# JuliaCrypto/ToyFHE.jl

Measured on AMD Instinct MI355X. Metric: ciphertext-mul/s (BFV ct*ct + relinearize, N=2^14, L=8 RNS), higher is better.
Workload: dtype u64; 1 GPU; BFV N=2^14, L=8 RNS limbs (50-bit primes), extension basis 17 limbs, t=65537, ciphertext-mul + relinearize (RNS-digit keyswitch), bit-exact; batch_per_gpu=1024, global_batch=1024

## Files before the change

toyfhe.jl_amd/csrc/bfv_api.inc:

```

struct tfhe_bfv_plan {
    tfhe_ctx *small = nullptr, *big = nullptr;
    limb_sel_t sel_s, sel_b;
    u64 t = 0;
    bfv_tab_t tab;
    bfv_tab_t* tab_dev = nullptr;
    std::vector<void*> allocs;
    int chunk = 256;
    void* ws = nullptr;
    size_t ws_bytes = 0;
    bool relin_ok = false;
    bfv_fast_tab_t* fast_dev = nullptr;
    int fast_ns = 0, fast_np = 0;
    bool fast_narrow = false;
    bool use_fast = true;
    hipEvent_t order_ev = nullptr;
};

namespace {

int upload(tfhe_bfv_plan* p, const std::vector<u64>& v, const u64** out) {
    void* d = nullptr;
    hipError_t e = devalloc::malloc_retry(&d, std::max<size_t>(8, v.size() * 8));
    if (e != hipSuccess) return fail(TFHE_E_HIP, "hipMalloc: %s", hipGetErrorString(e));
// ... 187 lines not shown
    if (p->big && p->big->stream) hipStreamSynchronize(p->big->stream);
    if (p->small && p->small->stream && (!p->big || p->small->stream != p->big->stream)) hipStreamSynchronize(p->small->stream);
    if (p->order_ev) hipEventDestroy(p->order_ev);
    for (void* d : p->allocs) hipFree(d);
    if (p->tab_dev) hipFree(p->tab_dev);
    if (p->fast_dev) hipFree(p->fast_dev);
    if (p->ws) hipFree(p->ws);
    delete p;
    return TFHE_OK;
}

int tfhe_bfv_plan_set_chunk(tfhe_bfv_plan* p, int chunk) {
    if (!p || chunk < 0) return fail(TFHE_E_BADARG, "bad argument");
    p->chunk = chunk ? chunk : 256;
    return TFHE_OK;
}

int tfhe_bfv_plan_set_variant(tfhe_bfv_plan* p, int variant) {
    if (!p || variant < 0 || variant > 1) return fail(TFHE_E_BADARG, "variant must be 0 (auto) or 1 (general kernels)");
    p->use_fast = (variant == 0);
    return TFHE_OK;
}

int tfhe_bfv_expand(tfhe_bfv_plan* p, const uint64_t* src, uint64_t* dst, int64_t count) {
    if (!p || !src || !dst || count < 0) return fail(TFHE_E_BADARG, "bad argument");
    int rc = stream_order(p, p->small, p->big);
    if (!rc) rc = launch_expand(p, src, dst, count);
    if (!rc) rc = stream_order(p, p->big, p->small);
    return rc;
}
int tfhe_bfv_contract(tfhe_bfv_plan* p, const uint64_t* src, uint64_t* dst, int64_t count) {
    if (!p || !src || !dst || count < 0) return fail(TFHE_E_BADARG, "bad argument");
    int rc = stream_order(p, p->small, p->big);
    if (!rc) rc = launch_contract(p, src, dst, count);
    if (!rc) rc = stream_order(p, p->big, p->small);
    return rc;
}

static int bfv_mul_impl(tfhe_bfv_plan* p, const u64* evk, int n_digits, const u64* c1, const u64* c2, u64* out, int64_t batch) {
    if (!p || !c1 || !c2 || !out || batch < 0) return fail(TFHE_E_BADARG, "bad argument");
    const size_t N = (size_t)p->big->N;
    const int ns = p->tab.ns, nb = p->tab.nb;
    const bool relin = evk != nullptr;
    if (relin) {
        if (!p->relin_ok) return fail(TFHE_E_UNSUPPORTED, "relinearisation needs ℛ = limbs 0..ns-1 of the small context");
        if (n_digits < ns) return fail(TFHE_E_PARAMS_MISMATCH, "evaluation key has %d components, need %d", n_digits, ns);
    }
    const int64_t chunk = std::max<int64_t>(1, std::min<int64_t>(batch, p->chunk));
    const bool prelift = relin && p->fast_dev && p->use_fast && p->fast_narrow && ks_prelift_ok(p->small, ns);
    const size_t ntt_tmp = p->big->logN > 14 ? (size_t)chunk * 4 * nb * N * 8 : 0;
    (void)ntt_tmp;
    void* ws = nullptr;
    const size_t scr_rows = (size_t)2 * std::max(256, p->big->num_cus);
    int rc = plan_ws(p, ((size_t)chunk * (7 * (size_t)nb + (relin ? 3 * (size_t)ns : 0)) + scr_rows) * N * 8, &ws);
    if (rc) return rc;
    u64* E = (u64*)ws;
    u64* T = E + (size_t)chunk * 4 * nb * N;
    u64* R = T + (size_t)chunk * 3 * nb * N;
    u64* SCR = R + (relin ? (size_t)chunk * 3 * ns * N : 0);
    for (int64_t b0 = 0; b0 < batch; b0 += chunk) {
        const int64_t nct = std::min(chunk, batch - b0);
        const u64* a = c1 + (size_t)b0 * 2 * ns * N;
        const u64* b = c2 + (size_t)b0 * 2 * ns * N;
        rc = stream_order(p, p->small, p->big);
        if (rc) return rc;
        if (!relin) {
            rc = bfv_mul_chunk(p, a, b, out + (size_t)b0 * 3 * ns * N, nct, E, T, SCR);
            if (rc) return rc;
        } else {
            rc = bfv_mul_chunk(p, a, b, R, nct, E, T, SCR, prelift);
            if (!rc) rc = stream_order(p, p->big, p->small);
            if (rc) return rc;
            rc = keyswitch_impl(p->small, ns, ns, 0, evk, R, 3, out + (size_t)b0 * 2 * ns * N, nct, 0, false, prelift);
            if (rc) return rc;
        }
    }
    return relin ? TFHE_OK : stream_order(p, p->big, p->small);
}

int tfhe_bfv_mul(tfhe_bfv_plan* p, const uint64_t* c1, const uint64_t* c2, uint64_t* out, int64_t batch) {
    return bfv_mul_impl(p, nullptr, 0, c1, c2, out, batch);
}
int tfhe_bfv_mul_relin(tfhe_bfv_plan* p, const uint64_t* evk, int n_digits, const uint64_t* c1, const uint64_t* c2, uint64_t* out, int64_t batch) {
    if (!evk) return fail(TFHE_E_BADARG, "null evaluation key");
    return bfv_mul_impl(p, evk, n_digits, c1, c2, out, batch);
}

}
```

toyfhe.jl_amd/csrc/kernels.h:

```cpp
#pragma once
#include <hip/hip_runtime.h>
#include <type_traits>
#include "bfv_core.h"
#include "bfv_fast.h"
#include "lazy_sum.h"
#include "ntt_core.h"

typedef u64 u64x2_t __attribute__((ext_vector_type(2)));

#ifndef TFHE_NTT_WAVES
#define TFHE_NTT_WAVES 2
#endif

__device__ __forceinline__ u32 fresh_tid() {
    u32 t = threadIdx.x;
    asm volatile("" : "+v"(t));
    return t;
}

struct limb_sel_t {
    int n;
    int idx[TFHE_MAX_LIMBS];
};

// ... 67 lines not shown
        return item < nitems ? item : ~0u;
    }
    const u32 per = (nitems + 7u) >> 3, nslots = grid >> 3, xcd = wg & 7u, slot = wg >> 3;
    const u32 k = it * nslots + slot, idx = xcd * per + k;
    if (k >= per || idx >= nitems) return ~0u;
    const u32 B = nitems / nb, j = idx / B, b = idx - j * B;
    return b * nb + j;
}
__device__ __forceinline__ u32 dense_mask(u32 limbs, u32 mask) { return (limbs & 1u) ? 0u : mask; }
__device__ __forceinline__ u32 dense_count(u32 nitems, int x, u32 limbs, u32 mask) {
    return mask ? ((((nitems >> x) / limbs) * (u32)__popc(mask)) << x) : nitems;
}
__device__ __forceinline__ u32 dense_item(u32 d, int x, u32 limbs, u32 mask) {
    if (!mask || d == ~0u) return d;
    const u32 nact = (u32)__popc(mask), sb = d & ((1u << x) - 1u), pld = d >> x, g = pld / nact, a = pld % nact;
    u32 m = mask;
    for (u32 i = 0; i < a; i++) m &= m - 1u;
    return ((g * limbs + (u32)__ffs((int)m) - 1u) << x) | sb;
}
template <class A, int LOGB, int LOGT, int IOMODE>
__global__ __launch_bounds__(1 << LOGT, TFHE_NTT_WAVES) void k_ntt_fwd_block(const u64* __restrict__ src, u64* __restrict__ dst,
                                                              const ntt_limb_t* __restrict__ LT, limb_sel_t sel, int x,
                                                              u32 nitems, ntt_io_t io) {
    extern __shared__ __attribute__((aligned(16))) u64 lds[];
    const size_t ntot = (size_t)1 << (LOGB + x);
    const u32 dmask = dense_mask((u32)sel.n, io.limb_mask), dn = dense_count(nitems, x, (u32)sel.n, dmask), niter = (dn + gridDim.x - 1) / gridDim.x;
    bool first = true;
    for (u32 it = 0; it < niter; it++) {
        const u32 item = dense_item(xcd_walk_item(it, blockIdx.x, gridDim.x, x, dn), x, (u32)sel.n, dmask);
        if (item == ~0u) continue;
        const u32 sb = item & ((1u << x) - 1), pl = item >> x;
        u32 srow = pl, drow = pl, j = pl % (u32)sel.n;
        lift_t lf;
        const lift_t* lift = nullptr;
        if constexpr (IOMODE == 1) {
            const u32 per_ct = io.level * io.nw, b = pl / per_ct, rem = pl % per_ct, i = rem / io.nw;
            j = rem % io.nw;
            srow = (b * io.polys + io.polys - 1) * io.level + i;
            const ntt_limb_t& Li = LT[sel.idx[i]];
            const ntt_limb_t& Lj = LT[sel.idx[j]];
            lf.qi = Li.q; lf.half = Li.q >> 1; lf.qj = Lj.q; lf.bj = Lj.br;
            if (io.lift_unsigned) lf.qi = lf.half = ~0ull;
            lift_wide_consts<A>(lf);
            lift = &lf;
        }
        if (io.limb_mask && !((io.limb_mask >> j) & 1u)) continue;
        const typename A::ctx C = A::make(LT[sel.idx[j]]);
        if (!first) __syncthreads();
        first = false;
        fwd_schedule<A, LOGB, LOGT, 0>(lds, src + srow * ntot + ((size_t)sb << LOGB), dst + drow * ntot, C, fresh_tid(),
                                       (1u << x) + sb, x, brev_bits(sb, x), lift);
    }
}
template <class T>
__device__ __forceinline__ void pin_vgpr(T& x) { asm volatile("" : "+v"(x)); }
__device__ __forceinline__ void order_after(u32& idx, u64 v) { asm volatile("" : "+v"(idx) : "v"(v)); }
#define TFHE_WAIT_VM0() asm volatile("s_waitcnt vmcnt(0)" ::: "memory")
template <int LOGB, int LOGT>
struct row_prefetcher {
    static constexpr int E = 1 << (LOGB - LOGT);
    u64* raw;
    const u64* g;
    bool on;
    __device__ __forceinline__ void operator()(int before, int after, int total) const {
        const int lo2 = 2 * E * before / total, hi2 = 2 * E * after / total;
        const int lo = lo2 < E ? lo2 : E, hi = hi2 < E ? hi2 : E;
        if (hi > lo && on) {
#pragma unroll
            for (int i = lo; i < hi; i++) raw[i] = g[(size_t)i << LOGT];
        }
    }
};
template <class A, int LOGB, int LOGT>
__global__ __launch_bounds__(1 << LOGT, TFHE_NTT_WAVES) void k_ntt_fwd_pf(const u64* __restrict__ src, u64* __restrict__ dst,
                                                           const ntt_limb_t* __restrict__ LT, limb_sel_t sel, u32 nitems) {
    extern __shared__ __attribute__((aligned(16))) u64 lds[];
    constexpr int K1 = pass_k_fwd(LOGB, LOGT, 0), K2 = pass_k_fwd(LOGB, LOGT, K1), K3 = LOGB - K1 - K2;
    static_assert(K3 >= 1 && pass_k_fwd(LOGB, LOGT, K1 + K2) == K3, "three-pass schedule expected");
    typedef pgeom<LOGB, LOGT, K1, K2> G2;
    typedef pgeom<LOGB, LOGT, K1 + K2, K3> G3;
    static_assert(G2::SETS == 1, "middle pass: one register set");
    constexpr int E = G3::E;
    u32 item = blockIdx.x;
    if (item >= nitems) return;
    u64 raw[E];
    fwd_load_data<LOGB, LOGT, 0, K1, true, false>(raw, lds, src + ((size_t)item << LOGB), threadIdx.x);
    for (bool first = true;; first = false) {
        const u32 tid = fresh_tid();
        const typename A::ctx C = A::make(LT[sel.idx[item % (u32)sel.n]]);
        u64* gdst = dst + ((size_t)item << LOGB);
        const u32 next = item + gridDim.x;
        if (!first) __syncthreads();
        typename A::tw tw2[G2::SETS * G2::NTW];
        {
            typename A::elem v[E];
            fwd_compute<A, LOGB, LOGT, 0, K1, true, false, 0>(v, raw, nullptr, C, tid, 1u);
            fwd_load_tw<A, LOGB, LOGT, K1, K2, false>(tw2, C, tid, 1u);
            fwd_store<A, LOGB, LOGT, 0, K1, false>(v, lds, nullptr, C, tid, 0, 0u);
        }
        __syncthreads();
        {
            u64 r2[E];
            typename A::elem v[E];
            fwd_load_data<LOGB, LOGT, K1, K2, false, false>(r2, lds, nullptr, tid);
#pragma unroll
            for (int i = 0; i < G2::SETS * G2::NTW; i++) pin_vgpr(tw2[i].w);
            const row_prefetcher<LOGB, LOGT> pf{raw, src + ((size_t)(next < nitems ? next : item) << LOGB) + tid, next < nitems};
            fwd_compute<A, LOGB, LOGT, K1, K2, false, false, K2, -1, row_prefetcher<LOGB, LOGT>>(v, r2, tw2, C, tid, 1u, nullptr, pf);
// ... 1163 lines not shown
            u64x2_t p1 = {0, 0}, p2 = {0, 0};
            if (i0) {
                p1 = *s1p; p2 = *s2p;
                if (pairs) { const u64x2_t a = p1, c = p2; p1.x = a.x; p1.y = c.x; p2.x = a.y; p2.y = c.y; }
            }
            acc52 s1[2] = {{p1[0], 0, 0}, {p1[1], 0, 0}}, s2[2] = {{p2[0], 0, 0}, {p2[1], 0, 0}};
            u64x2_t dv[DCH];
#pragma unroll
            for (int ii = 0; ii < DCH; ii++)
                if (i0 + ii < A.level) dv[ii] = *(const u64x2_t*)(dig + (((size_t)b * A.level + i0 + ii) * A.nw + j) * n + k);
#pragma unroll
            for (int ii = 0; ii < DCH; ii++) {
                if (i0 + ii < A.level) {
#pragma unroll
                    for (int v = 0; v < 2; v++) {
                        const u32 d0 = (u32)dv[ii][v] & 0x3ffffffu, d1 = (u32)(dv[ii][v] >> 26);
                        acc52_mac(s1[v], d0, d1, md0[ii][v], md1[ii][v]);
                        acc52_mac(s2[v], d0, d1, mk0[ii][v], mk1[ii][v]);
                    }
                }
            }
            u64x2_t r1, r2;
#pragma unroll
            for (int v = 0; v < 2; v++) {
                u64 lo, hi;
                acc52_fold(s1[v], lo, hi);
                r1[v] = barrett_reduce128(lo, hi, br);
                acc52_fold(s2[v], lo, hi);
                r2[v] = barrett_reduce128(lo, hi, br);
            }
            if constexpr (EPI) {
                if (i0 + DCH >= A.level && j < (u32)A.level) {
                    const u64x2_t x = *(const u64x2_t*)(K.epi_x + (((size_t)b * 2) * A.level + j) * n + k);
#pragma unroll
                    for (int v = 0; v < 2; v++) {
                        r1[v] = addmod(shoup_full(r1[v], A.pinv[j], br.q), x[v], br.q);
                        r2[v] = shoup_full(r2[v], A.pinv[j], br.q);
                    }
                }
            }
            if (pairs) {
                u64x2_t a, c;
                a.x = r1[0]; a.y = r2[0]; c.x = r1[1]; c.y = r2[1];
                *s1p = a;
                *s2p = c;
            } else {
                *s1p = r1;
                *s2p = r2;
            }
        }
    }
}

template <class A, int LOGB, int LOGT, bool PRELIFT = false>
__device__ __forceinline__ void fused_fwd_to_regs(u64* lds, const u64* grow, const typename A::ctx& C, bool& first,
                                                  typename A::elem* v, const lift_t* lift = nullptr) {
    constexpr int K1 = pass_k_fwd(LOGB, LOGT, 0), K2 = pass_k_fwd(LOGB, LOGT, K1), K3 = LOGB - K1 - K2;
    constexpr int E = 1 << (LOGB - LOGT);
    const u32 tid = fresh_tid();
    {
        u64 raw[E];
        fwd_load_data<LOGB, LOGT, 0, K1, true, false>(raw, lds, grow, tid);
        if (!first) __syncthreads();
        first = false;
        if constexpr (PRELIFT) {
#pragma unroll
            for (int i = 0; i < E; i++) pin_vgpr(raw[i]);
            TFHE_SCHED_FENCE();
            fwd_compute<A, LOGB, LOGT, 0, K1, false, false, 0>(v, raw, nullptr, C, tid, 1u);
        } else {
            fwd_compute<A, LOGB, LOGT, 0, K1, true, false, 0>(v, raw, nullptr, C, tid, 1u, lift);
        }
        fwd_store<A, LOGB, LOGT, 0, K1, false>(v, lds, nullptr, C, tid, 0, 0u);
    }
    __syncthreads();
    ntt_fwd_pass<A, LOGB, LOGT, K1, K2, false, false>(lds, nullptr, nullptr, C, tid, 1u, 0, 0u);
    __syncthreads();
    {
        u64 r3[E];
        fwd_load_data<LOGB, LOGT, K1 + K2, K3, false, true>(r3, lds, nullptr, tid);
        fwd_compute<A, LOGB, LOGT, K1 + K2, K3, false, true, 0>(v, r3, nullptr, C, tid, 1u);
    }
}
template <class A, int LOGB, int LOGT, bool SCALE = true, class AO = A>
__device__ __forceinline__ void fused_inv_from_regs(u64* lds, typename A::elem* v, u64* gdst, const typename A::ctx& C, const u64* addend,
                                                    u64* keep = nullptr, u32 pre = 1u) {
    constexpr int KI1 = pass_k_inv(LOGB, LOGT, LOGB);
    constexpr int E = 1 << (LOGB - LOGT);
    const u32 tid = fresh_tid();
    __syncthreads();
    constexpr int S1 = LOGB - KI1, K2 = pass_k_inv(LOGB, LOGT, S1);
    typedef pgeom<LOGB, LOGT, S1 - K2, K2> G2;
    typename A::tw tw_next[G2::SETS * G2::NTW];
    {
#pragma unroll
        for (int e = 0; e < E; e++) v[e] = fp_reduce(v[e], C.p, C.pinv);
        inv_compute<A, LOGB, LOGT, S1, KI1, true, SCALE, 0, -1, no_hook, true>(v, nullptr, nullptr, C, tid, pre);
        if constexpr (S1 - K2 != 0) inv_load_tw<A, LOGB, LOGT, S1 - K2, K2, false>(tw_next, C, tid, pre);
        inv_store<A, LOGB, LOGT, S1, KI1, true, SCALE>(v, lds, nullptr, C, tid);
    }
    __syncthreads();
    inv_schedule_ptw<A, LOGB, LOGT, S1, SCALE, AO>(lds, nullptr, gdst, C, tid, pre, addend, tw_next, keep);
}

template <class A, int LOGB, int LOGT>
__global__ __launch_bounds__(1 << LOGT) void k_ntt_inv_quad2(const u64* __restrict__ src, u64* __restrict__ dst,
                                                              const ntt_limb_t* __restrict__ LT, limb_sel_t sel, u32 nitems, u32 limb_mask) {
    extern __shared__ __attribute__((aligned(16))) u64 lds[];
    constexpr int x = 2;
    constexpr int K1 = pass_k_inv(LOGB, LOGT, LOGB), S1 = LOGB - K1;
    typedef pgeom<LOGB, LOGT, S1, K1> G1;
    constexpr int E = G1::E;
    constexpr int K2 = pass_k_inv(LOGB, LOGT, S1), KL = S1 - K2;
    static_assert(KL >= 1 && pass_k_inv(LOGB, LOGT, KL) == KL, "three-pass schedule expected");
    typedef pgeom<LOGB, LOGT, 0, KL> GL;
    static_assert(GL::SETS == 1 && GL::LO == LOGT, "last pass: element r of a thread is word tid + (r << LOGT)");
    static_assert(G1::SETS << (LOGT + K1) == 1 << LOGB, "first pass: register position e <-> point tid + (e << LOGT)");
    const size_t ntot = (size_t)1 << (LOGB + x);
// ... 62 lines not shown
                    for (int r = 0; r < E; r++) held[r] = A::out_inv_scaled(v[r], C);
                } else {
#pragma unroll
                    for (int r = 0; r < E; r++) {
                        u64x2_t ww;
                        ww.x = held[r];
                        ww.y = A::out_inv_scaled(v[r], C);
                        *(u64x2_t*)(d + ((u64)(tid + ((u32)r << LOGT)) << x)) = ww;
                    }
                }
            }
        }
    }
}

__global__ __launch_bounds__(256) void k_evk_to_f64(const u64* __restrict__ evk, u64* __restrict__ evd,
                                                     const ntt_limb_t* __restrict__ LT, ks_arg_t KA, int Lk, u32 n, int fold_ninv, int x,
                                                     u64 ginv, int pair) {
    const u32 row = blockIdx.x, j = row % (u32)KA.nw, ic = row / (u32)KA.nw;
    const ntt_limb_t& L = LT[KA.w.idx[j]];
    const u64* s = evk + ((size_t)ic * Lk + KA.w.idx[j]) * n;
    u64* d = pair ? evd + (((size_t)(ic >> 1) * KA.nw + j) * n) * 2 + (ic & 1u) : evd + (size_t)row * n;
    for (u32 k = blockIdx.y * blockDim.x + threadIdx.x; k < n; k += gridDim.y * blockDim.x) {
        double v = fp_from_u64(s[ginv ? galois_ntt_pos(k, ginv, n) : k]);
        if (fold_ninv) {
            v = fp_mulmod_c(v, L.ninv_d, L.pd, L.pinvd);
            v = v < 0.0 ? v + L.pd : v;
        }
        u64 b;
        __builtin_memcpy(&b, &v, 8);
        const size_t pos = x ? ((size_t)(k & ((1u << x) - 1u)) * (n >> x)) + (k >> x) : (size_t)k;
        d[pair ? pos * 2 : pos] = b;
    }
}
template <int LOGB, int LOGT>
constexpr size_t fused_lds_bytes() {
    return (size_t)lds_words<LOGB, LOGT>() * 8;
}
template <class A, int LOGB, int LOGT, bool PRELIFT = false, int SPMODE = 0>
__global__ __launch_bounds__(1 << LOGT) void k_ks_fused(const u64* __restrict__ evd, const u64* __restrict__ ct,
                                                         u64* __restrict__ out, const ntt_limb_t* __restrict__ LT,
                                                         ks_arg_t KA, int Lk, u32 nitems, const u64* __restrict__ tsp = nullptr,
                                                         const u64* __restrict__ zero_row = nullptr) {
    extern __shared__ __attribute__((aligned(16))) u64 lds[];
    constexpr int K1 = pass_k_fwd(LOGB, LOGT, 0), K2 = pass_k_fwd(LOGB, LOGT, K1), K3 = LOGB - K1 - K2;
    static_assert(K3 >= 1 && pass_k_fwd(LOGB, LOGT, K1 + K2) == K3, "three-pass forward schedule expected");
    constexpr int KI1 = pass_k_inv(LOGB, LOGT, LOGB);
    static_assert(KI1 == K3, "forward last pass and inverse first pass must share the register map");
    typedef pgeom<LOGB, LOGT, 0, K1> G1;
    typedef pgeom<LOGB, LOGT, K1 + K2, K3> G3;
    constexpr int E = G3::E;
    const u32 level = (u32)KA.level, polys = (u32)KA.polys, nw = (u32)KA.nw;
    const u32 add_s = polys == 3 ? 2u : 1u;
    bool first = true;
    const u32 niter = (nitems + gridDim.x - 1) / gridDim.x;
    for (u32 it = 0; it < niter; it++) {
        const u32 nper = SPMODE == 1 ? 1u : (SPMODE >= 2 ? level : nw);
        const u32 item = it * gridDim.x + blockIdx.x;
        if (item >= nitems) break;
        const u32 b = item / nper, j = SPMODE == 1 ? level : item % nper;
        const ntt_limb_t& Lj = LT[KA.w.idx[j]];
        typename A::ctx C = A::make(Lj);
        lift_t lf;
        lf.qj = Lj.q;
        lf.bj = Lj.br;
        typename A::elem acc[2][E];
#pragma unroll
        for (int e = 0; e < E; e++) acc[0][e] = acc[1][e] = 0;
        for (u32 i = 0; i < level; i++) {
            const u32 tid = fresh_tid();
            lf.qi = LT[KA.w.idx[i]].q;
            lf.half = lf.qi >> 1;
            const u64* grow = ct + ((size_t)((b * polys + polys - 1) * level + i) << LOGB);
            typename A::elem v[E];
            fused_fwd_to_regs<A, LOGB, LOGT, PRELIFT>(lds, grow, C, first, v, &lf);
            const u64x2_t* e_pair = (const u64x2_t*)(evd + ((((size_t)i * nw + j) << LOGB) << 1));
#pragma unroll
            for (int u = 0; u < G3::SETS; u++) {
                u32 c0, hi, base;
                G3::template coords<true>(tid, u, c0, hi, base);
#pragma unroll
                for (int r = 0; r < G3::R; r++) {
                    const u32 nat = (brev_bits((u32)r, K3) << (LOGB - K3)) + c0;
                    const int e = u * G3::R + r;
                    const u64x2_t kw = e_pair[nat];
                    const typename A::tw k1{A::from_lds(kw.y)}, k0{A::from_lds(kw.x)};
                    const double y = A::pre_product(v[e], C);
                    acc[0][e] += fp_mulmod_c(y, k1, C.p, C.pinv);
                    acc[1][e] += fp_mulmod_c(y, k0, C.p, C.pinv);
                }
            }
            if ((i & 7u) == 7u && i + 1 < level) {
#pragma unroll
                for (int e = 0; e < E; e++) {
                    acc[0][e] = fp_reduce(acc[0][e], C.p, C.pinv);
                    acc[1][e] = fp_reduce(acc[1][e], C.p, C.pinv);
                }
            }
        }
#pragma unroll
        for (int sidx = 0; sidx < 2; sidx++) {
            if constexpr (SPMODE >= 2) {
                C.md_pinv = (double)KA.pinv[j].w;
                C.md_c = (u32)sidx < add_s ? ct + ((size_t)((b * polys + sidx) * level + j) << LOGB) : zero_row;
                C.md_g = KA.rot_g;
                u64* gdst = out + ((size_t)((b * 2 + sidx) * level + j) << LOGB);
                typedef typename std::conditional<SPMODE == 3, ArithFpMDR, ArithFpMD>::type AOUT;
                fused_inv_from_regs<A, LOGB, LOGT, false, AOUT>(lds, acc[sidx], gdst, C, tsp + ((size_t)(b * 2 + sidx) << LOGB));
            } else if constexpr (SPMODE == 1) {
                u64* gdst = out + ((size_t)(b * 2 + sidx) << LOGB);
                fused_inv_from_regs<A, LOGB, LOGT, false>(lds, acc[sidx], gdst, C, nullptr);
            } else {
                const u64* addend = (!KA.special && (u32)sidx < add_s) ? ct + ((size_t)((b * polys + sidx) * level + j) << LOGB) : nullptr;
                u64* gdst = out + ((size_t)((b * 2 + sidx) * nw + j) << LOGB);
                fused_inv_from_regs<A, LOGB, LOGT, false>(lds, acc[sidx], gdst, C, addend);
            }
        }
    }
}

template <class A, int LOGB, int LOGT, int X>
__global__ __launch_bounds__(1 << LOGT) void k_ks_fused_sub(const u64* __restrict__ evd, const u64* __restrict__ ct,
                                                             u64* __restrict__ T, const ntt_limb_t* __restrict__ LT,
                                                             ks_arg_t KA, int Lk, u32 nitems) {
    extern __shared__ __attribute__((aligned(16))) u64 lds[];
    constexpr int K1 = pass_k_fwd(LOGB, LOGT, 0), K2 = pass_k_fwd(LOGB, LOGT, K1), K3 = LOGB - K1 - K2;
    static_assert(K3 >= 1 && pass_k_fwd(LOGB, LOGT, K1 + K2) == K3, "three-pass forward schedule expected");
    constexpr int KI1 = pass_k_inv(LOGB, LOGT, LOGB), S1 = LOGB - KI1;
// ... 671 lines not shown
```

toyfhe.jl_amd/csrc/ks_api.inc:

```

static bool ks_fused14(const tfhe_ctx* c, int Lk, int level, int special) {
    const limb_sel_t w = working_limbs(Lk, level, special);
    if (c->variant != 0) return false;
    if (c->logN == 14) return sel_fp(c, w, 0);
    if (c->logN == 13) {
        static const bool on = env_flag("TFHE_FUSED13", true);
        return on && sel_fp(c, w, 0);
    }
    if (c->logN == 16) {
        static const bool on16 = env_flag("TFHE_FUSED16", true);
        return on16 && level >= 2 && sel_fp(c, w, 2);
    }
    return c->logN == 15 && level >= 2 && sel_fp(c, w, 1);
}
static bool ks_prelift_ok(const tfhe_ctx* c, int level) {
    if (c->logN != 14 || !ks_fused14(c, level, level, 0)) return false;
    u64 lo = ~0ull, hi = 0;
    for (int j = 0; j < level; j++) { lo = std::min(lo, c->q[j]); hi = std::max(hi, c->q[j]); }
    return hi <= 2 * lo;
}
static int launch_top_lift(tfhe_ctx* c, const u64* src, u64* t, int64_t rows, const limb_sel_t& sel, const ntt_io_t& io) {
    const int x = c->logN - 14;
    const dim3 tg((unsigned)((((c->N >> x) + 255) / 256) * rows));
    return dispatch_int<1, 2>(x, [&](auto xc) {
// ... 233 lines not shown
                         : (P.fps ? k_ks_fused_sub<ArithFpS, 14, LOGT, 1> : k_ks_fused_sub<ArithFp, 14, LOGT, 1>);
        const unsigned items = (unsigned)((batch * nw) << x);
        rc = launch_prof(c, (int64_t)batch * nw * (level + 2), fk, dim3(cu_grid(c, items)), dim3(1 << LOGT), lds, key, ct, dig, c->limbs_dev, A, Lk, items);
        if (rc) return rc;
        return launch_top_tail(c, A, P.ra, dig, ct, out, batch, P.g_tail);
    }
    lanes_t outer(c, P.two_lanes);
    rc = ks_digits_fwd(c, A, ct, dig, batch);
    if (rc) return rc;
    rc = ks_inner_launch(c, A, Lk, key, dig, S, batch);
    if (rc) return rc;
    if (P.tail16) {
        const policy_split_t ps = policy_split(c, A.w);
        const u32 fpm = ps.fpmask, amask = ps.all;
        {
            lanes_t lanes(c, fpm != amask);
            lanes.use(1);
            rc = launch_subpair<ArithFp>(c, true, S, dig, batch * 2 * nw, A.w, 2, fpm == amask ? 0u : fpm);
            if (rc) return rc;
            if (fpm != amask) {
                lanes.use(0);
                ntt_io_t iw = io_plain();
                iw.limb_mask = amask & ~fpm;
                rc = launch_block_inv<ArithInt, 14>(c, S, dig, batch * 2 * nw, A.w, 2, iw);
                if (rc) return rc;
            }
        }
        outer.join();
        return launch_top_tail(c, A, P.ra, dig, ct, out, batch, P.g_tail);
    }
    outer.join();
    return ks_plain_tail(c, A, P.ra, S, ct, out, batch);
}

static int ks_check(tfhe_ctx* c, int Lk, int level, int special, const void* evk, int n_digits, const void* ct, int polys, const void* out, int64_t batch) {
    if (!c || !evk || !ct || !out) return fail(TFHE_E_BADARG, "null argument");
    if (polys != 2 && polys != 3) return fail(TFHE_E_BADARG, "keyswitch needs a 2- or 3-element ciphertext (rlwe_she.jl:318), got %d", polys);
    if (Lk < 1 || Lk > c->L) return fail(TFHE_E_LEVEL_MISMATCH, "key_limbs=%d outside [1,%d]", Lk, c->L);
    const int maxlevel = special ? Lk - 1 : Lk;
    if (level < 1 || level > maxlevel) return fail(TFHE_E_LEVEL_MISMATCH, "level=%d outside [1,%d]", level, maxlevel);
    if (n_digits < level) return fail(TFHE_E_PARAMS_MISMATCH, "evaluation key has %d components, level %d needs %d", n_digits, level, level);
    if (batch < 0) return fail(TFHE_E_BADARG, "negative batch");
    return TFHE_OK;
}
static int galois_check(const tfhe_ctx* c, u64 g) {
    if ((g & 1) == 0 || g >= 2 * (u64)c->N) return fail(TFHE_E_BADARG, "galois element must be odd and below 2N");
    return TFHE_OK;
}
static u64 inv_mod_2n(u64 g, u64 twoN) {
    u64 x = g;
    for (int i = 0; i < 6; i++) x *= 2 - g * x;
    return x & (twoN - 1);
}
static int keyswitch_impl(tfhe_ctx* c, int Lk, int level, int special, const u64* evk, const u64* ct, int polys, u64* out, int64_t batch,
                          u64 galois, bool rotate, bool prelifted = false, bool key_prepared = false) {
    if (prelifted && (rotate || special || !ks_prelift_ok(c, level))) return fail(TFHE_E_UNSUPPORTED, "internal: pre-lifted rows need the fused key switch");
    ks_plan_t P = ks_plan(c, Lk, level, special, polys, batch, ct, out, galois, rotate, prelifted, key_prepared);
    if (P.rot == KS_ROT_HOISTED) {
        const uint64_t* one[1] = {evk};
        return tfhe_rotate_many(c, Lk, level, special, one, level, 1, &galois, 1, ct, out, batch);
    }
    if (special) special_inv_table(c, Lk, level, P.ra.qlinv);
    const size_t N = P.N;
    void* ws = nullptr;
    int rc = ensure_ws(c, P.bytes(), &ws);
    if (rc) return rc;
    u64 *const S = P.region(ws, 0), *const dig = P.region(ws, P.S_rows), *const rot = P.region(ws, P.S_rows + P.dig_rows),
        *const kw = P.region(ws, P.S_rows + P.dig_rows + P.rot_rows);
    const u64 ginv = P.key_perm ? inv_mod_2n(galois, 2 * (u64)c->N) : (u64)0;
    if (P.path != KS_THREE) {
        rc = launch(c, k_evk_to_f64, row_grid((unsigned)(level * 2 * P.A.nw), N), dim3(256), 0, evk, kw, c->limbs_dev, P.A, Lk, (u32)N, c->logN <= 14 ? 1 : 0,
                    c->logN == 16 ? 2 : 0, ginv, 1);
    } else if (P.key_perm) {
        rc = launch(c, k_ntt_perm, row_grid((unsigned)(level * 2 * Lk), N), dim3(256), 0, evk, kw, ginv, (u32)N);
    }
    if (rc) return rc;
    if (P.path != KS_THREE || P.key_perm) evk = kw;
    for (int64_t b0 = 0; b0 < batch; b0 += P.chunk) {
        const int64_t nb = std::min(P.chunk, batch - b0);
        const u64* cin = ct + (size_t)b0 * polys * level * N;
        if (P.rot == KS_ROT_COPY) {
            rc = do_galois(c, cin, rot, galois, nb * polys * level, first_limbs(level));
            if (rc) return rc;
            cin = rot;
        }
        rc = ks_chunk(c, P, evk, cin, out + (size_t)b0 * 2 * level * N, nb, S, dig);
        if (rc) return rc;
    }
    return TFHE_OK;
}

int tfhe_keyswitch(tfhe_ctx* c, int Lk, int level, int special, const uint64_t* evk, int n_digits, const uint64_t* ct, int polys, uint64_t* out, int64_t batch) {
    int rc = ks_check(c, Lk, level, special, evk, n_digits, ct, polys, out, batch);
    if (rc) return rc;
    return keyswitch_impl(c, Lk, level, special, evk, ct, polys, out, batch, 0, false);
}
int tfhe_galois_key_prepare(tfhe_ctx* c, int Lk, int n_digits, uint64_t g, const uint64_t* evk, uint64_t* evk_out) {
    if (!c || !evk || !evk_out || evk == evk_out) return fail(TFHE_E_BADARG, "null or aliased argument");
    if (Lk < 1 || Lk > c->L || n_digits < 1) return fail(TFHE_E_LEVEL_MISMATCH, "key shape outside the ring");
    if (int rc = galois_check(c, g)) return rc;
    const u64 ginv = inv_mod_2n(g, 2 * (u64)c->N);
    return launch(c, k_ntt_perm, row_grid((unsigned)(n_digits * 2 * Lk), (size_t)c->N), dim3(256), 0, evk, evk_out, ginv, (u32)c->N);
}

struct rotate_many_ws_t {
    size_t per_ct, ntt_tmp;
    int64_t chunk;
    size_t bytes() const { return ntt_tmp + (size_t)chunk * per_ct; }
};
static rotate_many_ws_t rotate_many_ws(const tfhe_ctx* c, int level, int nw, int64_t batch) {
    rotate_many_ws_t W{};
    W.per_ct = ((size_t)4 * nw + (size_t)level * nw + (size_t)2 * level) * (size_t)c->N * 8;
    W.chunk = chunk_of(c, batch, 512, (size_t)8192 << 20, W.per_ct);
    W.ntt_tmp = c->logN > 14 ? (size_t)W.chunk * std::max(2, level) * nw * (size_t)c->N * 8 : 0;
    return W;
}
int tfhe_rotate_many(tfhe_ctx* c, int Lk, int level, int special, const uint64_t* const* evks, int n_digits, int prepared,
                     const uint64_t* galois, int n_rot, const uint64_t* ct, uint64_t* out, int64_t batch) {
    if (!evks || !galois || n_rot < 0) return fail(TFHE_E_BADARG, "null argument");
    if (n_rot == 0) return TFHE_OK;
    for (int r = 0; r < n_rot; r++) {
        int rc = ks_check(c, Lk, level, special, evks[r], n_digits, ct, 2, out, batch);
        if (!rc) rc = galois_check(c, galois[r]);
        if (rc) return rc;
    }
    const int nw = special ? level + 1 : level, polys = 2;
    const size_t N = (size_t)c->N;
    if (!prepared && c->logN <= 14 && ks_fused14(c, Lk, level, special)) {
        for (int r = 0; r < n_rot; r++) {
            int rc = keyswitch_impl(c, Lk, level, special, evks[r], ct, 2, out + (size_t)r * batch * 2 * level * N, batch, galois[r], true);
// ... 154 lines not shown
```

toyfhe.jl_amd/csrc/ntt_core.h:

```cpp
#pragma once
#include "fp64arith.h"
#include "modarith.h"

#if defined(__HIP_DEVICE_COMPILE__)
#define TFHE_SCHED_FENCE() asm volatile("" ::: "memory")
#else
#define TFHE_SCHED_FENCE() ((void)0)
#endif

struct alignas(16) twd_t {
    u64 w, wp;
};
TFHE_HD tw_t as_tw(const twd_t& t) { return tw_t{t.w, t.wp}; }
TFHE_HD tw_t ld_tw(const twd_t* tab, u32 i) {
#if defined(__HIP_DEVICE_COMPILE__)
    typedef __attribute__((address_space(1))) const twd_t* gptr_t;
    const gptr_t g = (gptr_t)tab;
    return tw_t{g[i].w, g[i].wp};
#else
    return tw_t{tab[i].w, tab[i].wp};
#endif
}

template <int LOGB, int LOGT>
TFHE_HD u32 lds_phi(u32 j) {
    if (LOGB - LOGT == 5) return j + 2u * (j >> 6) + (j >> 10);
    return j + 4u * (j >> 6) + (j >> 9);
}
template <int LOGB, int LOGT>
constexpr u32 lds_phi_c(u32 j) {
    return (LOGB - LOGT == 5) ? (j + 2u * (j >> 6) + (j >> 10)) : (j + 4u * (j >> 6) + (j >> 9));
}
template <int LOGB, int LOGT>
constexpr u32 lds_words() {
    constexpr u32 m = (1u << LOGB) - 1;
    return (LOGB - LOGT == 5) ? (m + 2u * (m >> 6) + (m >> 10) + 1) : (m + 4u * (m >> 6) + (m >> 9) + 1);
}
constexpr int logt_for(int logb) { return logb >= 13 ? logb - 5 : logb - 4; }
constexpr int pass_k_fwd(int logb, int logt, int s0) { return (logb - s0) >= (logb - logt) ? (logb - logt) : (logb - s0); }
constexpr int pass_k_inv(int logb, int logt, int s_end) { return (s_end % (logb - logt)) ? (s_end % (logb - logt)) : (logb - logt); }

TFHE_HD void bfly_fwd(u64& x, u64& y, tw_t w, u64 q) {
    u64 u = csub_s(x, 2 * q);
    u64 t = shoup_lazy(y, w, q);
    x = u + t;
    y = u + 2 * q - t;
}
TFHE_HD void bfly_inv(u64& x, u64& y, tw_t w, u64 q) {
    u64 a = csub_s(x + y, 2 * q);
    u64 d = x + 2 * q - y;
    x = a;
    y = shoup_lazy(d, w, q);
}

struct ntt_limb_t {
    u64 q;
    tw_t ninv;
    tw_t w1inv_ninv;
    barrett_t br;
    const twd_t* W;
    const twd_t* Winv;
// ... 67 lines not shown
constexpr bool fp_fwd_sweep_before(int nstages, int s) {
    double b = 1.0;
    for (int t = 0; t < nstages; t++) {
        const bool sweep = b * (1.0 + 1.5 * TFHE_FP_A) + 0.5 > TFHE_FP_LIMIT;
        if (t == s) return sweep;
        if (sweep) b = 0.5001;
        b = b * (1.0 + 1.5 * TFHE_FP_A) + 0.5;
    }
    return false;
}
struct ArithFp {
    static constexpr bool prefetch_tw = true;
    static constexpr bool moddown = false;
    static constexpr bool fwd_sweep_before(int nstages, int s) { return fp_fwd_sweep_before(nstages, s); }
    static constexpr double fp_a = TFHE_FP_A, fp_lim = TFHE_FP_LIMIT;
    template <int LOGB, int LOGT, int S0> static constexpr bool inv_lds_reduce() { return true; }
    template <int LOGB, int LOGT, int SEND> static constexpr double inv_entry() { return 0.502; }
    typedef double elem;
    typedef ftw_t tw;
    struct ctx {
        double p, pinv;
        const ftwd_t *W, *Winv, *Wb, *Winvb;
        ftw_t ninv, w1n;
        u64 q;
        double md_pinv = 0.0;
        const u64* md_c = nullptr;
        u32 md_g = 0;
    };
    static TFHE_HD ctx make(const ntt_limb_t& L) {
        return ctx{L.pd, L.pinvd, L.Wd, L.Winvd, L.Wdb, L.Winvdb, L.ninv_d, L.w1inv_ninv_d, L.q};
    }
    static TFHE_HD elem from_global(u64 x, const ctx& c) {
        const double d = fp_from_u64(x);
        return d + d > c.p ? d - c.p : d;
    }
    static TFHE_HD elem from_global_plain(u64 x, const ctx&) { return fp_from_u64(x); }
    static TFHE_HD elem from_global_lift(u64 x, const ctx& c, const lift_t& f, bool loose = false) {
        double d = fp_from_u64(x);
        d = x > f.half ? d - (double)f.qi : d;
        return (loose && f.qi <= 2 * c.q) ? d : fp_reduce(d, c.p, c.pinv);
    }
    static TFHE_HD elem from_lds(u64 x) { double d; __builtin_memcpy(&d, &x, 8); return d; }
    static TFHE_HD u64 to_lds(elem v) { u64 b; __builtin_memcpy(&b, &v, 8); return b; }
    static TFHE_HD tw ld(const ftwd_t* tab, u32 i) {
#if defined(__HIP_DEVICE_COMPILE__)
        typedef __attribute__((address_space(1))) const ftwd_t* gptr_t;
        const gptr_t g = (gptr_t)tab;
        return ftw_t{g[i]};
#else
        return ftw_t{tab[i]};
#endif
    }
    static TFHE_HD tw ld_fwd(const ctx& c, u32 i) { return ld(c.W, i); }
    static TFHE_HD tw ld_inv(const ctx& c, u32 i) { return ld(c.Winv, i); }
    static TFHE_HD tw ld_fwd_b(const ctx& c, u32 i) { return ld(c.Wb, i); }
    static TFHE_HD tw ld_inv_b(const ctx& c, u32 i) { return ld(c.Winvb, i); }
    static TFHE_HD bool has_b(const ctx& c) { return c.Wb != nullptr; }
    static TFHE_HD void bf_fwd(elem& x, elem& y, tw w, const ctx& c) {
        const double t = fp_mulmod_c(y, w, c.p, c.pinv);
        y = x - t;
        x = x + t;
    }
    static TFHE_HD void bf_inv(elem& x, elem& y, tw w, const ctx& c) {
        const double a = x + y, d = x - y;
        x = a;
        y = fp_mulmod_c(d, w, c.p, c.pinv);
    }
    static TFHE_HD void bf_inv_scaled(elem& x, elem& y, const ctx& c) {
        const double a = x + y, d = x - y;
        x = fp_mulmod_c(a, c.ninv, c.p, c.pinv);
        y = fp_mulmod_c(d, c.w1n, c.p, c.pinv);
    }
    static TFHE_HD void range_fwd(elem& v, const ctx& c) { v = fp_reduce(v, c.p, c.pinv); }
    static TFHE_HD void range_inv(elem& v, const ctx& c) { v = fp_reduce(v, c.p, c.pinv); }
    static TFHE_HD elem pre_product(elem v, const ctx& c) { return fp_reduce(v, c.p, c.pinv); }
    static TFHE_HD elem top_reduce(elem v, const ctx& c) { return fp_reduce(v, c.p, c.pinv); }
    static TFHE_HD u64 out_fwd(elem v, const ctx& c) { return fp_canon(v, c.p, c.pinv); }
    static TFHE_HD u64 out_inv_scaled(elem v, const ctx& c) { return fp_canon(v, c.p, c.pinv); }
    static TFHE_HD u64 out_inv_lazy(elem v, const ctx& c) { return fp_canon(v, c.p, c.pinv); }
};
struct ArithFpD : ArithFp {
    static TFHE_HD u64 out_inv_scaled(elem v, const ctx& c) { return to_lds(fp_reduce(v, c.p, c.pinv)); }
    static TFHE_HD u64 out_inv_lazy(elem v, const ctx& c) { return to_lds(fp_reduce(v, c.p, c.pinv)); }
};
struct ArithFpMD : ArithFp {
    static constexpr bool moddown = true;
    static constexpr bool rot = false;
    static TFHE_HD u64 out_moddown(elem v, u64 tsp, u64 cw, const ctx& c) {
        const double x = fp_reduce(v, c.p, c.pinv) - fp_reduce(fp_from_u64(tsp), c.p, c.pinv);
        return fp_canon(fp_mulmod_c(x, ftw_t{c.md_pinv}, c.p, c.pinv) + fp_from_u64(cw), c.p, c.pinv);
    }
};
struct ArithFpMDR : ArithFpMD {
    static constexpr bool rot = true;
    static TFHE_HD u64 out_moddown_rot(elem v, u64 tsp, u64 cw, bool neg, const ctx& c) {
        const double x = fp_reduce(v, c.p, c.pinv) - fp_reduce(fp_from_u64(tsp), c.p, c.pinv);
        const double y = fp_mulmod_c(x, ftw_t{c.md_pinv}, c.p, c.pinv) + fp_from_u64(cw);
        return fp_canon(neg ? -y - (tsp != 0 ? 1.0 : 0.0) : y, c.p, c.pinv);
    }
};
struct ArithFpWide : ArithFp {
    static TFHE_HD elem from_global_lift(u64 x, const ctx& c, const lift_t& f, bool = false) {
        const double dl = (double)(u32)x, dh = (double)(u32)(x >> 32);
        double r = fp_mulmod_c(dh, ftw_t{f.c32}, c.p, c.pinv) + dl;
        r = x > f.half ? r - f.qim : r;
        return fp_reduce(r, c.p, c.pinv);
// ... 105 lines not shown
        for (int r = 0; r < G::R; r++) {
            const u32 j = base + ((u32)r << G::LO);
            raw[u * G::R + r] = FIRST ? gsrc[j] : xchg_rd(lds, pb + lds_phi_c<LOGB, LOGT>((u32)r << G::LO));
        }
    }
    TFHE_SCHED_FENCE();
    (void)lift;
}
template <class A, int LOGB, int LOGT, int S0, int K, bool FIRST, bool LAST, int PF, int USEL = -1, class HOOK = no_hook>
TFHE_HD void fwd_compute(typename A::elem* v, const u64* raw, const typename A::tw* twp, const typename A::ctx& C, u32 tid,
                         u32 pre, const lift_t* lift = nullptr, const HOOK& hook = HOOK(), u64* lds_early = nullptr) {
    typedef pgeom<LOGB, LOGT, S0, K> G;
    const bool use_b = LAST && A::has_b(C);
    if (FIRST && lift) {
#pragma unroll
        for (int i = 0; i < G::E; i++) v[i] = A::from_global_lift(raw[i], C, *lift, true);
        TFHE_SCHED_FENCE();
    }
#pragma unroll
    for (int u = 0; u < G::SETS; u++) {
        if (USEL >= 0 && u != USEL) continue;
        u32 c0, hi, base;
        G::template coords<LAST>(tid, u, c0, hi, base);
        typename A::elem* vv = v + u * G::R;
#pragma unroll
        for (int r = 0; r < G::R; r++) {
            if (FIRST && lift) continue;
            vv[r] = FIRST ? A::from_global_plain(raw[u * G::R + r], C) : A::from_lds(raw[u * G::R + r]);
        }
#pragma unroll
        for (int d = 0; d < K; d++) {
            const int half = 1 << (K - 1 - d);
            if (A::fwd_sweep_before(LOGB, S0 + d)) {
#pragma unroll
                for (int r = 0; r < G::R; r++) A::range_fwd(vv[r], C);
            }
#pragma unroll
            for (int g = 0; g < (1 << d); g++) {
                const typename A::tw w = d < PF ? twp[u * G::NTW + (1 << d) - 1 + g]
                                         : (LAST && use_b) ? A::ld_fwd_b(C, (pre << (S0 + d)) + (c0 << d) + (u32)g)
                                                           : A::ld_fwd(C, (pre << (S0 + d)) + (hi << d) + (u32)g);
#pragma unroll
                for (int i = 0; i < half; i++) {
                    const int r0 = (g << (K - d)) + i;
                    A::bf_fwd(vv[r0], vv[r0 + half], w, C);
                    if (!LAST && lds_early && d == K - 1) {
                        const u32 pb = lds_phi<LOGB, LOGT>(base);
                        xchg_wr(lds_early, pb + lds_phi_c<LOGB, LOGT>((u32)r0 << G::LO), A::to_lds(vv[r0]));
                        xchg_wr(lds_early, pb + lds_phi_c<LOGB, LOGT>((u32)(r0 + 1) << G::LO), A::to_lds(vv[r0 + 1]));
                    }
                }
                hook(((u * K + d) * (G::R / 2)) + g * half, ((u * K + d) * (G::R / 2)) + (g + 1) * half, G::SETS * K * (G::R / 2));
            }
        }
    }
}
template <class A, int LOGB, int LOGT, int S0, int K, bool LAST, int USEL = -1>
TFHE_HD void fwd_store(typename A::elem* v, u64* lds, u64* gdst, const typename A::ctx& C, u32 tid, int x, u32 sb_rev) {
    typedef pgeom<LOGB, LOGT, S0, K> G;
    static_assert(!LAST || G::LO == 0, "LAST pass must end at stage LOGB-1");
#pragma unroll
    for (int u = 0; u < G::SETS; u++) {
        if (USEL >= 0 && u != USEL) continue;
        u32 c0, hi, base;
        G::template coords<LAST>(tid, u, c0, hi, base);
        const u32 pb = LAST ? 0u : lds_phi<LOGB, LOGT>(base);
#pragma unroll
        for (int r = 0; r < G::R; r++) {
            typename A::elem e = v[u * G::R + r];
            if (LAST) {
                const u32 nat = (brev_bits((u32)r, K) << (LOGB - K)) + c0;
                gdst[((u64)nat << x) + sb_rev] = A::out_fwd(e, C);
            } else {
                xchg_wr(lds, pb + lds_phi_c<LOGB, LOGT>((u32)r << G::LO), A::to_lds(e));
            }
        }
    }
}
template <class A, int LOGB, int LOGT, int S0, int K, bool FIRST, bool LAST, bool ES = false>
TFHE_HD void ntt_fwd_pass(u64* lds, const u64* gsrc, u64* gdst, const typename A::ctx& C, u32 tid, u32 pre, int x,
                          u32 sb_rev, const lift_t* lift = nullptr) {
    typedef pgeom<LOGB, LOGT, S0, K> G;
    u64 raw[G::E];
    typename A::elem v[G::E];
    fwd_load_data<LOGB, LOGT, S0, K, FIRST, LAST>(raw, lds, gsrc, tid);
    if constexpr (!LAST && ES) {
        fwd_compute<A, LOGB, LOGT, S0, K, FIRST, LAST, 0>(v, raw, nullptr, C, tid, pre, FIRST ? lift : nullptr, no_hook(), lds);
    } else {
        fwd_compute<A, LOGB, LOGT, S0, K, FIRST, LAST, 0>(v, raw, nullptr, C, tid, pre, FIRST ? lift : nullptr);
        fwd_store<A, LOGB, LOGT, S0, K, LAST>(v, lds, gdst, C, tid, x, sb_rev);
    }
}

template <class A, int LOGB, int LOGT, int S0, int K, bool FROM_GLOBAL, int D0 = 0, int D1 = K>
TFHE_HD void inv_load_tw(typename A::tw* tw, const typename A::ctx& C, u32 tid, u32 pre) {
    typedef pgeom<LOGB, LOGT, S0, K> G;
#pragma unroll
    for (int u = 0; u < G::SETS; u++) {
        u32 c0, hi, base;
        G::template coords<FROM_GLOBAL>(tid, u, c0, hi, base);
#pragma unroll
        for (int d = D0; d < D1; d++)
#pragma unroll
            for (int g = 0; g < (1 << d); g++)
                tw[u * G::NTW + (1 << d) - 1 + g] = A::ld_inv(C, (pre << (S0 + d)) + (hi << d) + (u32)g);
    }
// ... 279 lines not shown
```

Measured before the change: 63420 ciphertext-mul/s.

## Split first NTT pass into load classes and hoist key conversion out of chunk loop

The first forward NTT pass in the fused keyswitch (FP64, N=2^14, prelifted) now loads its rows in four interleaved classes. Butterflies on each class start while later loads are still in flight, and twiddles are read through the scalar constant address space. Separately, the evaluation key conversion to f64 or permuted form now runs once per multiply call into a workspace region, instead of once per chunk inside keyswitch_impl. This trades extra workspace and more register pressure for less per-chunk conversion work and better overlap of memory latency with compute.

```diff
diff --git a/toyfhe.jl_amd/csrc/bfv_api.inc b/toyfhe.jl_amd/csrc/bfv_api.inc
--- a/toyfhe.jl_amd/csrc/bfv_api.inc
+++ b/toyfhe.jl_amd/csrc/bfv_api.inc
@@ -263,12 +263,19 @@
     (void)ntt_tmp;
     void* ws = nullptr;
     const size_t scr_rows = (size_t)2 * std::max(256, p->big->num_cus);
-    int rc = plan_ws(p, ((size_t)chunk * (7 * (size_t)nb + (relin ? 3 * (size_t)ns : 0)) + scr_rows) * N * 8, &ws);
+    const ks_plan_t KP = relin ? ks_plan(p->small, ns, ns, 0, 3, chunk, nullptr, nullptr, 0, false, prelift) : ks_plan_t{};
+    const size_t key_bytes = (relin && batch > 0 && ks_key_converted(KP)) ? KP.key_bytes : 0;
+    int rc = plan_ws(p, ((size_t)chunk * (7 * (size_t)nb + (relin ? 3 * (size_t)ns : 0)) + scr_rows) * N * 8 + key_bytes, &ws);
     if (rc) return rc;
     u64* E = (u64*)ws;
     u64* T = E + (size_t)chunk * 4 * nb * N;
     u64* R = T + (size_t)chunk * 3 * nb * N;
     u64* SCR = R + (relin ? (size_t)chunk * 3 * ns * N : 0);
+    u64* KW = key_bytes ? SCR + scr_rows * N : nullptr;
+    if (KW) {
+        rc = ks_convert_key(p->small, KP, evk, KW, 0);
+        if (rc) return rc;
+    }
     for (int64_t b0 = 0; b0 < batch; b0 += chunk) {
         const int64_t nct = std::min(chunk, batch - b0);
         const u64* a = c1 + (size_t)b0 * 2 * ns * N;
@@ -282,7 +289,7 @@
             rc = bfv_mul_chunk(p, a, b, R, nct, E, T, SCR, prelift);
             if (!rc) rc = stream_order(p, p->big, p->small);
             if (rc) return rc;
-            rc = keyswitch_impl(p->small, ns, ns, 0, evk, R, 3, out + (size_t)b0 * 2 * ns * N, nct, 0, false, prelift);
+            rc = keyswitch_impl(p->small, ns, ns, 0, evk, R, 3, out + (size_t)b0 * 2 * ns * N, nct, 0, false, prelift, false, KW);
             if (rc) return rc;
         }
     }
diff --git a/toyfhe.jl_amd/csrc/kernels.h b/toyfhe.jl_amd/csrc/kernels.h
--- a/toyfhe.jl_amd/csrc/kernels.h
+++ b/toyfhe.jl_amd/csrc/kernels.h
@@ -143,8 +143,6 @@
                                        (1u << x) + sb, x, brev_bits(sb, x), lift);
     }
 }
-template <class T>
-__device__ __forceinline__ void pin_vgpr(T& x) { asm volatile("" : "+v"(x)); }
 __device__ __forceinline__ void order_after(u32& idx, u64 v) { asm volatile("" : "+v"(idx) : "v"(v)); }
 #define TFHE_WAIT_VM0() asm volatile("s_waitcnt vmcnt(0)" ::: "memory")
 template <int LOGB, int LOGT>
@@ -1414,7 +1412,7 @@
     }
 }
 
-template <class A, int LOGB, int LOGT, bool PRELIFT = false>
+template <class A, int LOGB, int LOGT, bool PRELIFT = false, int NC = 0>
 __device__ __forceinline__ void fused_fwd_to_regs(u64* lds, const u64* grow, const typename A::ctx& C, bool& first,
                                                   typename A::elem* v, const lift_t* lift = nullptr) {
     constexpr int K1 = pass_k_fwd(LOGB, LOGT, 0), K2 = pass_k_fwd(LOGB, LOGT, K1), K3 = LOGB - K1 - K2;
@@ -1422,10 +1420,13 @@
     const u32 tid = fresh_tid();
     {
         u64 raw[E];
-        fwd_load_data<LOGB, LOGT, 0, K1, true, false>(raw, lds, grow, tid);
+        if constexpr (NC != 0) fwd_load_data_split<LOGB, LOGT, K1, NC>(raw, grow, tid);
+        else fwd_load_data<LOGB, LOGT, 0, K1, true, false>(raw, lds, grow, tid);
         if (!first) __syncthreads();
         first = false;
-        if constexpr (PRELIFT) {
+        if constexpr (NC != 0) {
+            fwd_compute_split<A, LOGB, LOGT, K1, NC, PRELIFT>(v, raw, C, 1u, lift);
+        } else if constexpr (PRELIFT) {
 #pragma unroll
             for (int i = 0; i < E; i++) pin_vgpr(raw[i]);
             TFHE_SCHED_FENCE();
@@ -1594,6 +1595,7 @@
     constexpr int E = G3::E;
     const u32 level = (u32)KA.level, polys = (u32)KA.polys, nw = (u32)KA.nw;
     const u32 add_s = polys == 3 ? 2u : 1u;
+    constexpr int FNC = (std::is_same<A, ArithFp>::value && LOGB == 14 && PRELIFT && SPMODE == 0) ? TFHE_FIRST_PASS_NC : 0;
     bool first = true;
     const u32 niter = (nitems + gridDim.x - 1) / gridDim.x;
     for (u32 it = 0; it < niter; it++) {
@@ -1615,7 +1617,7 @@
             lf.half = lf.qi >> 1;
             const u64* grow = ct + ((size_t)((b * polys + polys - 1) * level + i) << LOGB);
             typename A::elem v[E];
-            fused_fwd_to_regs<A, LOGB, LOGT, PRELIFT>(lds, grow, C, first, v, &lf);
+            fused_fwd_to_regs<A, LOGB, LOGT, PRELIFT, FNC>(lds, grow, C, first, v, &lf);
             const u64x2_t* e_pair = (const u64x2_t*)(evd + ((((size_t)i * nw + j) << LOGB) << 1));
 #pragma unroll
             for (int u = 0; u < G3::SETS; u++) {
diff --git a/toyfhe.jl_amd/csrc/ks_api.inc b/toyfhe.jl_amd/csrc/ks_api.inc
--- a/toyfhe.jl_amd/csrc/ks_api.inc
+++ b/toyfhe.jl_amd/csrc/ks_api.inc
@@ -309,10 +309,23 @@
     for (int i = 0; i < 6; i++) x *= 2 - g * x;
     return x & (twoN - 1);
 }
+static bool ks_key_converted(const ks_plan_t& P) { return P.path != KS_THREE || P.key_perm; }
+static int ks_convert_key(tfhe_ctx* c, const ks_plan_t& P, const u64* evk, u64* kw, u64 galois) {
+    const size_t N = P.N;
+    const int level = P.A.level;
+    const u64 ginv = P.key_perm ? inv_mod_2n(galois, 2 * (u64)c->N) : (u64)0;
+    if (P.path != KS_THREE)
+        return launch(c, k_evk_to_f64, row_grid((unsigned)(level * 2 * P.A.nw), N), dim3(256), 0, evk, kw, c->limbs_dev, P.A, P.Lk, (u32)N, c->logN <= 14 ? 1 : 0,
+                      c->logN == 16 ? 2 : 0, ginv, 1);
+    if (P.key_perm) return launch(c, k_ntt_perm, row_grid((unsigned)(level * 2 * P.Lk), N), dim3(256), 0, evk, kw, ginv, (u32)N);
+    return TFHE_OK;
+}
 static int keyswitch_impl(tfhe_ctx* c, int Lk, int level, int special, const u64* evk, const u64* ct, int polys, u64* out, int64_t batch,
-                          u64 galois, bool rotate, bool prelifted = false, bool key_prepared = false) {
+                          u64 galois, bool rotate, bool prelifted = false, bool key_prepared = false, const u64* key_rows = nullptr) {
     if (prelifted && (rotate || special || !ks_prelift_ok(c, level))) return fail(TFHE_E_UNSUPPORTED, "internal: pre-lifted rows need the fused key switch");
+    if (key_rows && rotate) return fail(TFHE_E_UNSUPPORTED, "internal: converted key rows are for plain key switches");
     ks_plan_t P = ks_plan(c, Lk, level, special, polys, batch, ct, out, galois, rotate, prelifted, key_prepared);
+    if (key_rows) P.key_bytes = 0;
     if (P.rot == KS_ROT_HOISTED) {
         const uint64_t* one[1] = {evk};
         return tfhe_rotate_many(c, Lk, level, special, one, level, 1, &galois, 1, ct, out, batch);
@@ -324,15 +337,13 @@
     if (rc) return rc;
     u64 *const S = P.region(ws, 0), *const dig = P.region(ws, P.S_rows), *const rot = P.region(ws, P.S_rows + P.dig_rows),
         *const kw = P.region(ws, P.S_rows + P.dig_rows + P.rot_rows);
-    const u64 ginv = P.key_perm ? inv_mod_2n(galois, 2 * (u64)c->N) : (u64)0;
-    if (P.path != KS_THREE) {
-        rc = launch(c, k_evk_to_f64, row_grid((unsigned)(level * 2 * P.A.nw), N), dim3(256), 0, evk, kw, c->limbs_dev, P.A, Lk, (u32)N, c->logN <= 14 ? 1 : 0,
-                    c->logN == 16 ? 2 : 0, ginv, 1);
-    } else if (P.key_perm) {
-        rc = launch(c, k_ntt_perm, row_grid((unsigned)(level * 2 * Lk), N), dim3(256), 0, evk, kw, ginv, (u32)N);
-    }
-    if (rc) return rc;
-    if (P.path != KS_THREE || P.key_perm) evk = kw;
+    if (ks_key_converted(P)) {
+        if (!key_rows) {
+            rc = ks_convert_key(c, P, evk, kw, galois);
+            if (rc) return rc;
+        }
+        evk = key_rows ? key_rows : kw;
+    }
     for (int64_t b0 = 0; b0 < batch; b0 += P.chunk) {
         const int64_t nb = std::min(P.chunk, batch - b0);
         const u64* cin = ct + (size_t)b0 * polys * level * N;
diff --git a/toyfhe.jl_amd/csrc/ntt_core.h b/toyfhe.jl_amd/csrc/ntt_core.h
--- a/toyfhe.jl_amd/csrc/ntt_core.h
+++ b/toyfhe.jl_amd/csrc/ntt_core.h
@@ -7,6 +7,19 @@
 #else
 #define TFHE_SCHED_FENCE() ((void)0)
 #endif
+#if defined(__HIP_DEVICE_COMPILE__)
+#define TFHE_SCHED_BARRIER() __builtin_amdgcn_sched_barrier(0)
+#else
+#define TFHE_SCHED_BARRIER() ((void)0)
+#endif
+template <class T>
+TFHE_HD void pin_vgpr(T& x) {
+#if defined(__HIP_DEVICE_COMPILE__)
+    asm volatile("" : "+v"(x));
+#else
+    (void)x;
+#endif
+}
 
 struct alignas(16) twd_t {
     u64 w, wp;
@@ -180,6 +193,14 @@
 #endif
     }
     static TFHE_HD tw ld_fwd(const ctx& c, u32 i) { return ld(c.W, i); }
+    static TFHE_HD tw ld_fwd_uniform(const ctx& c, u32 i) {
+#if defined(__HIP_DEVICE_COMPILE__)
+        typedef __attribute__((address_space(4))) const ftwd_t* cptr_t;
+        return ftw_t{((cptr_t)c.W)[i]};
+#else
+        return ftw_t{c.W[i]};
+#endif
+    }
     static TFHE_HD tw ld_inv(const ctx& c, u32 i) { return ld(c.Winv, i); }
     static TFHE_HD tw ld_fwd_b(const ctx& c, u32 i) { return ld(c.Wb, i); }
     static TFHE_HD tw ld_inv_b(const ctx& c, u32 i) { return ld(c.Winvb, i); }
@@ -391,6 +412,66 @@
                 }
                 hook(((u * K + d) * (G::R / 2)) + g * half, ((u * K + d) * (G::R / 2)) + (g + 1) * half, G::SETS * K * (G::R / 2));
             }
+        }
+    }
+}
+constexpr int TFHE_FIRST_PASS_NC = 4;
+template <int LOGB, int LOGT, int K, int NC>
+TFHE_HD void fwd_load_data_split(u64* raw, const u64* gsrc, u32 tid) {
+    typedef pgeom<LOGB, LOGT, 0, K> G;
+    static_assert(G::SETS == 1 && G::LO >= LOGT, "one register set with workgroup-uniform twiddles (a FIRST pass)");
+    static_assert((NC == 2 || NC == 4) && NC < G::R, "two or four classes");
+    u32 c0, hi, base;
+    G::template coords<false>(tid, 0, c0, hi, base);
+#pragma unroll
+    for (int c = 0; c < NC; c++) {
+#pragma unroll
+        for (int r = c; r < G::R; r += NC) raw[r] = gsrc[base + ((u32)r << G::LO)];
+        TFHE_SCHED_BARRIER();
+    }
+    TFHE_SCHED_FENCE();
+}
+template <class A, int LOGB, int LOGT, int K, int NC, bool BITS>
+TFHE_HD void fwd_compute_split(typename A::elem* v, u64* raw, const typename A::ctx& C, u32 pre, const lift_t* lift = nullptr) {
+    typedef pgeom<LOGB, LOGT, 0, K> G;
+    static_assert(G::SETS == 1 && G::LO >= LOGT, "one register set with workgroup-uniform twiddles (a FIRST pass)");
+    constexpr int KC = NC == 2 ? K - 1 : K - 2;
+#pragma unroll
+    for (int c = 0; c < NC; c++) {
+#pragma unroll
+        for (int r = c; r < G::R; r += NC) pin_vgpr(raw[r]);
+        TFHE_SCHED_FENCE();
+#pragma unroll
+        for (int r = c; r < G::R; r += NC)
+            v[r] = BITS ? A::from_lds(raw[r]) : lift ? A::from_global_lift(raw[r], C, *lift, true) : A::from_global_plain(raw[r], C);
+#pragma unroll
+        for (int d = 0; d < KC; d++) {
+            const int half = 1 << (K - 1 - d);
+            if (A::fwd_sweep_before(LOGB, d)) {
+#pragma unroll
+                for (int r = c; r < G::R; r += NC) A::range_fwd(v[r], C);
+            }
+#pragma unroll
+            for (int g = 0; g < (1 << d); g++) {
+                const typename A::tw w = A::ld_fwd_uniform(C, (pre << d) + (u32)g);
+#pragma unroll
+                for (int i = c; i < half; i += NC) A::bf_fwd(v[(g << (K - d)) + i], v[(g << (K - d)) + i + half], w, C);
+            }
+        }
+        TFHE_SCHED_BARRIER();
+    }
+#pragma unroll
+    for (int d = KC; d < K; d++) {
+        const int half = 1 << (K - 1 - d);
+        if (A::fwd_sweep_before(LOGB, d)) {
+#pragma unroll
+            for (int r = 0; r < G::R; r++) A::range_fwd(v[r], C);
+        }
+#pragma unroll
+        for (int g = 0; g < (1 << d); g++) {
+            const typename A::tw w = A::ld_fwd_uniform(C, (pre << d) + (u32)g);
+#pragma unroll
+            for (int i = 0; i < half; i++) A::bf_fwd(v[(g << (K - d)) + i], v[(g << (K - d)) + i + half], w, C);
         }
     }
 }
```

Result: no change. 64000 ciphertext-mul/s (median of 6 runs) (+0.9%).
